# PRBonn/SHINE_mapping

Hardware: NVIDIA H100
Metric: sdf_train_points_per_sec_fwd_bwd (higher is better)
Workload: dtype f32

## Files before the change

### shine_mapping_b200/csrc/shine_b200.cu

```cuda

#include <cuda_runtime.h>
#include <math.h>
#include <stdint.h>

#include "shine_b200.h"

#ifndef SHINE_SECTOR_PROBE_TRAIN
#define SHINE_SECTOR_PROBE_TRAIN 0
#endif
#ifndef SHINE_SECTOR_PROBE_INFER
#define SHINE_SECTOR_PROBE_INFER 1
#endif
#ifndef SHINE_CPASYNC_PREFETCH
#define SHINE_CPASYNC_PREFETCH 0
#endif
#ifndef SHINE_GATHER_GROUP
#define SHINE_GATHER_GROUP 2
#endif
#ifndef SHINE_SLOT_PREFETCH
#define SHINE_SLOT_PREFETCH 0
#endif
#ifndef SHINE_ZERO_TILE_SKIP
#define SHINE_ZERO_TILE_SKIP 1
#endif
// ... 205 lines not shown
    }
    float g3[3] = {0.f, 0.f, 0.f};
    float4 acc = make_float4(0.f, 0.f, 0.f, 0.f);
    for (int i = 0; i < oct.num_levels; ++i) {
        const shine_level& lv = oct.lv[i];
        const HashSlot* slots = reinterpret_cast<const HashSlot*>(lv.hash_slots);
        const int s = valid ? probe_slot(slots, lv.hash_capacity - 1, morton_of(x, y, z, lv.level)) : -1;
        if (s < 0) continue;
        const int4 ia = ldg_i4(slots[s].ids0), ib = ldg_i4(slots[s].ids1);
        const int ids[8] = {ia.x, ib.x, ia.y, ib.y, ia.z, ib.z, ia.w, ib.w};
        BlendD b; b.init(x, y, z, lv.level, oct.poly_interp != 0);
#pragma unroll
        for (int c = 0; c < 8; ++c) {
            float g[3]; b.dw(c, g);
            if (MODE == 0) {
                const float4 v = ldg_f4(lv.features + (int64_t)ids[c] * F + 4 * part);
                const float q = v.x * d.x + v.y * d.y + v.z * d.z + v.w * d.w;
                g3[0] = fmaf(g[0], q, g3[0]); g3[1] = fmaf(g[1], q, g3[1]); g3[2] = fmaf(g[2], q, g3[2]);
            } else {
                const float w = tg[0] * g[0] + tg[1] * g[1] + tg[2] * g[2];
                if (MODE == 1) {
                    const float4 v = ldg_f4(lv.features + (int64_t)ids[c] * F + 4 * part);
                    acc.x = fmaf(w, v.x, acc.x); acc.y = fmaf(w, v.y, acc.y); acc.z = fmaf(w, v.z, acc.z); acc.w = fmaf(w, v.w, acc.w);
                } else {
                    red_add_f4(lv.feature_grads + (int64_t)ids[c] * F + 4 * part, w * d.x, w * d.y, w * d.z, w * d.w);
                }
            }
        }
    }
    if (MODE == 0) {
#pragma unroll
        for (int o = 1; o < LP; o <<= 1) {
            g3[0] += __shfl_xor_sync(kFull, g3[0], o); g3[1] += __shfl_xor_sync(kFull, g3[1], o); g3[2] += __shfl_xor_sync(kFull, g3[2], o);
        }
        if (valid && part == 0) { out[3 * p] = g3[0]; out[3 * p + 1] = g3[1]; out[3 * p + 2] = g3[2]; }
    } else if (MODE == 1) {
        if (valid) *reinterpret_cast<float4*>(out + p * F + 4 * part) = acc;
    }
}

__device__ __forceinline__ void to_afrag(const float (&v)[4], int odd, float (&a)[4]) {
    const float s0 = odd ? v[0] : v[2], s1 = odd ? v[1] : v[3];
    const float r0 = __shfl_xor_sync(kFull, s0, 1), r1 = __shfl_xor_sync(kFull, s1, 1);
    if (!odd) { a[0] = v[0]; a[2] = v[1]; a[1] = r0; a[3] = r1; }
    else      { a[0] = r0;   a[2] = r1;   a[1] = v[2]; a[3] = v[3]; }
}
__device__ __forceinline__ void from_cfrag(const float (&c)[4], int odd, float (&v)[4]) {
    const float s0 = odd ? c[0] : c[2], s1 = odd ? c[1] : c[3];
    const float r0 = __shfl_xor_sync(kFull, s0, 1), r1 = __shfl_xor_sync(kFull, s1, 1);
    if (!odd) { v[0] = c[0]; v[1] = c[1]; v[2] = r0; v[3] = r1; }
    else      { v[0] = r0;   v[1] = r1;   v[2] = c[2]; v[3] = c[3]; }
}

__device__ __forceinline__ void reduce_scatter_g(const float (&v)[24], float (&out)[3], int lane) {
    float a[12], b[6];
    const bool b4 = (lane & 16) != 0, b3 = (lane & 8) != 0, b2 = (lane & 4) != 0;
#pragma unroll
    for (int i = 0; i < 12; ++i) a[i] = (b4 ? v[12 + i] : v[i]) + __shfl_xor_sync(kFull, b4 ? v[i] : v[12 + i], 16);
#pragma unroll
    for (int i = 0; i < 6; ++i) b[i] = (b3 ? a[6 + i] : a[i]) + __shfl_xor_sync(kFull, b3 ? a[i] : a[6 + i], 8);
#pragma unroll
    for (int i = 0; i < 3; ++i) out[i] = (b2 ? b[3 + i] : b[i]) + __shfl_xor_sync(kFull, b2 ? b[i] : b[3 + i], 4);
}

#define SHINE_ACC_DECL float dW2[2][4][4], dW1[2][4], db2p[4][2], db1p[4][2], dw3p[4][2]

__device__ __forceinline__ void round_bar(int id) { asm volatile("bar.sync %0, 256;" ::"r"(id) : "memory"); }


constexpr int kGatherGroup = SHINE_GATHER_GROUP;

using shine_internal::StepParams;

struct SmemPlan {
    static constexpr int W1 = 0;
    static constexpr int W1T = W1 + 2 * kH * kF;
    static constexpr int W2 = W1T + 2 * kF * kWS;
    static constexpr int W2T = W2 + 2 * kH * kWS;
    static constexpr int B1 = W2T + 2 * kH * kWS;
    static constexpr int B2 = B1 + kH;
    static constexpr int W3 = B2 + kH;
    static constexpr int B3 = W3 + kH;
    static constexpr int kDecGradFloats = kH * kF + kH + kH * kH + kH + kH + 1;
    static constexpr int RND = B3 + 4;
    static constexpr int PRE = RND + 8;
    static constexpr int kPrePerWarp = 5 * kTile;
    static constexpr int STAGE = PRE + 8 * kPrePerWarp;
    static constexpr int kStagePerWarp = 3 * kTile * kWS + kTile * kF;
    static constexpr int kGroupPerLevel = 4 * kTile;
};

constexpr int kMaxGroupedRuns = 6;

__device__ __forceinline__ void red_add_f2(float* p, float a, float b) {
    asm volatile("red.global.add.v2.f32 [%0], {%1,%2};" ::"l"(p), "f"(a), "f"(b) : "memory");
}
__device__ __forceinline__ int group_slot(int p) { return 4 * (p & 3) + (p >> 2); }

template <int LMAX>
__device__ __forceinline__ void grouped_scatter(const StepParams& P, int L, int tile, const float* __restrict__ pt,
                                                float* __restrict__ dtile, const float (&dxc)[4], int lane) {
    const int g = lane >> 2, t = lane & 3;
    *reinterpret_cast<float2*>(dtile + g * kF + 2 * t) = make_float2(dxc[0], dxc[1]);
    *reinterpret_cast<float2*>(dtile + (g + 8) * kF + 2 * t) = make_float2(dxc[2], dxc[3]);
    __syncwarp();
    uint2 bh[2], bl[2];
#pragma unroll
    for (int c = 0; c < 2; ++c)
        split_fast2(dtile[(8 * c + t) * kF + g], dtile[(8 * c + t + 4) * kF + g], bh[c].x, bh[c].y, bl[c].x, bl[c].y);
    const float sx = (g & 4) ? 1.f : -1.f, ox = (g & 4) ? 0.f : 1.f;
    const float sy = (g & 2) ? 1.f : -1.f, oy = (g & 2) ? 0.f : 1.f;
    const float sz = (g & 1) ? 1.f : -1.f, oz = (g & 1) ? 0.f : 1.f;
    const int id_off = 8 * (g & 1) + 4 + (g >> 1);
    const int own = group_slot(lane & 15);
#pragma unroll
    for (int i = 0; i < LMAX; ++i) {
        if (i >= L) break;
        const float* lt = pt + i * SmemPlan::kGroupPerLevel;
        const int v_own = __float_as_int(lt[48 + own]);
        const uint32_t same = __match_any_sync(kFull, v_own);
        const int lead = __ffs(same) - 1;
        const uint32_t bmask = __ballot_sync(kFull, v_own >= 0 && lead == lane);
        if (bmask == 0) continue;
        const int rid_own = v_own >= 0 ? __popc(bmask & ((1u << lead) - 1u)) : 255;
        const shine_level& lv = P.oct.lv[i];
        const int32_t* slot_words = reinterpret_cast<const int32_t*>(lv.hash_slots);
        float* gb = grad_base(lv, (uint32_t)tile, kF);
        const int nruns = __popc(bmask);
        if (nruns > kMaxGroupedRuns) {
            const int odd = t & 1, half = t >> 1, mp = group_slot(g + 8 * odd);
            const int v = __float_as_int(lt[48 + mp]);
            if (v >= 0) {
                const float tx = lt[mp], ty = lt[16 + mp], tz = lt[32 + mp];
                const float ux = __fsub_rn(1.0f, tx), uy = __fsub_rn(1.0f, ty), uz = __fsub_rn(1.0f, tz);
                const int4 e = ldg_i4(slot_words + 16 * (int64_t)v + 4), o = ldg_i4(slot_words + 16 * (int64_t)v + 12);
                const int ids[8] = {e.x, o.x, e.y, o.y, e.z, o.z, e.w, o.w};
                const float4 d = *reinterpret_cast<const float4*>(dtile + (g + 8 * odd) * kF + 4 * half);
                const float xy[4] = {__fmul_rn(ux, uy), __fmul_rn(ux, ty), __fmul_rn(tx, uy), __fmul_rn(tx, ty)};
                const f2_t zz = f2_pack(uz, tz), d01 = f2_pack(d.x, d.y), d23 = f2_pack(d.z, d.w);
#pragma unroll
                for (int c = 0; c < 8; c += 2) {
// ... 29 lines not shown
        uint32_t rem = bmask;
        for (int r = 0; r < nruns; r += 2) {
            const int p1 = __ffs(rem) - 1; rem &= rem - 1;
            const int p2 = rem ? __ffs(rem) - 1 : p1; rem &= rem - 1;
            const int v1 = __shfl_sync(kFull, v_own, p1);
            const int v2 = (r + 1 < nruns) ? __shfl_sync(kFull, v_own, p2) : -1;
            AFrag<3> a0, a1;
            a0.set(rid[0] == r ? w[0] : 0.f, rid[0] == r + 1 ? w[0] : 0.f, rid[1] == r ? w[1] : 0.f, rid[1] == r + 1 ? w[1] : 0.f);
            a1.set(rid[2] == r ? w[2] : 0.f, rid[2] == r + 1 ? w[2] : 0.f, rid[3] == r ? w[3] : 0.f, rid[3] == r + 1 ? w[3] : 0.f);
            float c0[4] = {0.f, 0.f, 0.f, 0.f}, c1[4] = {0.f, 0.f, 0.f, 0.f};
            mma3x2<3>(c0, c1, a0, a1, bh[0], bl[0], bh[1], bl[1]);
            if (v1 >= 0) {
                const int row = __ldg(slot_words + 16 * (int64_t)v1 + id_off);
                red_add_f2(gb + (int64_t)row * kF + 2 * t, c0[0] + c1[0], c0[1] + c1[1]);
            }
            if (v2 >= 0) {
                const int row = __ldg(slot_words + 16 * (int64_t)v2 + id_off);
                red_add_f2(gb + (int64_t)row * kF + 2 * t, c0[2] + c1[2], c0[3] + c1[3]);
            }
        }
    }
    __syncwarp();
}

template <int NTF, bool TRAIN, bool DEC_GRAD, int LMAX, bool GROUPED = false>
__global__ void __launch_bounds__(256, !TRAIN ? SHINE_INFER_MINB : (DEC_GRAD && !GROUPED) ? SHINE_TRAIN_DECGRAD_MINB : SHINE_TRAIN_MINB)
sdf_fused_kernel(const __grid_constant__ StepParams P) {
    static_assert(!GROUPED || TRAIN, "the grouped scatter belongs to the training kernels");
    static_assert(!DEC_GRAD || TRAIN, "decoder gradients belong to the training kernels");
    static_assert(SmemPlan::kStagePerWarp >= SmemPlan::kDecGradFloats, "a warp's staging area holds its partial decoder gradient");
    extern __shared__ __align__(16) float smem[];
    uint32_t* smu = reinterpret_cast<uint32_t*>(smem);
    const int tid = threadIdx.x, lane = tid & 31, warp = tid >> 5;
    const int g = lane >> 2, t = lane & 3, odd = t & 1, half = t >> 1;
    constexpr int kWarps = 8;

    for (int i = tid; i < kH * kF; i += blockDim.x) {
        const int nrow = i / kF, k = i % kF;
        uint32_t hi, lo; split_tf32(P.dec.w1[i], hi, lo);
        smu[SmemPlan::W1 + i] = hi; smu[SmemPlan::W1 + kH * kF + i] = lo;
        smu[SmemPlan::W1T + k * kWS + nrow] = hi; smu[SmemPlan::W1T + kF * kWS + k * kWS + nrow] = lo;
    }
    for (int i = tid; i < kH * kH; i += blockDim.x) {
        const int nrow = i / kH, k = i % kH;
        uint32_t hi, lo; split_tf32(P.dec.w2[i], hi, lo);
        smu[SmemPlan::W2 + nrow * kWS + k] = hi; smu[SmemPlan::W2 + kH * kWS + nrow * kWS + k] = lo;
        smu[SmemPlan::W2T + k * kWS + nrow] = hi; smu[SmemPlan::W2T + kH * kWS + k * kWS + nrow] = lo;
    }
    if (tid < kH) {
        smem[SmemPlan::B1 + tid] = P.dec.b1 ? P.dec.b1[tid] : 0.f;
        smem[SmemPlan::B2 + tid] = P.dec.b2 ? P.dec.b2[tid] : 0.f;
        smem[SmemPlan::W3 + tid] = P.dec.w3[tid];
    }
    if (tid == 0) smem[SmemPlan::B3] = P.dec.b3 ? P.dec.b3[0] : 0.f;
    constexpr int kPark = LMAX <= 4 ? 16 : 32;
    constexpr int kIdPark = 4 * LMAX;
    __syncthreads();
    SHINE_ACC_DECL;
#pragma unroll
    for (int a = 0; a < 2; ++a) {
#pragma unroll
        for (int b = 0; b < 4; ++b) { dW2[a][b][0] = dW2[a][b][1] = dW2[a][b][2] = dW2[a][b][3] = 0.f; }
        dW1[a][0] = dW1[a][1] = dW1[a][2] = dW1[a][3] = 0.f;
    }
#pragma unroll
    for (int j = 0; j < 4; ++j) { db2p[j][0] = db2p[j][1] = db1p[j][0] = db1p[j][1] = dw3p[j][0] = dw3p[j][1] = 0.f; }
    float dW2acc[4] = {0.f, 0.f, 0.f, 0.f}, dW1acc[4] = {0.f, 0.f, 0.f, 0.f};
    float vecacc[3] = {0.f, 0.f, 0.f};
    constexpr bool kRounds = DEC_GRAD && GROUPED;

    constexpr bool kSectorProbe = TRAIN ? (SHINE_SECTOR_PROBE_TRAIN != 0) : (SHINE_SECTOR_PROBE_INFER != 0);
    constexpr bool kSlotPrefetch = TRAIN && !kSectorProbe && (SHINE_SLOT_PREFETCH != 0) && (SHINE_CPASYNC_PREFETCH == 0);
    constexpr bool kZeroSkip = (SHINE_ZERO_TILE_SKIP != 0) && (SHINE_CPASYNC_PREFETCH == 0);
    const bool poly = P.oct.poly_interp != 0;
    const int L = P.oct.num_levels;
    const float up = (TRAIN && P.d_loss) ? __ldg(P.d_loss) : 1.0f;
    const float gscale = P.loss_scale * up;

    float db3p = 0.f;
    float loss_acc = 0.f;

    float* stage = smem + SmemPlan::STAGE + warp * SmemPlan::kStagePerWarp;
    float* stA = stage;
    float* stB = stage + kTile * kWS;
    float* stC = stage + 2 * kTile * kWS;
    float* stX = stage + 3 * kTile * kWS;
    float* gpt = smem + SmemPlan::STAGE + (DEC_GRAD ? 8 * SmemPlan::kStagePerWarp : 0) +
                 warp * (LMAX * SmemPlan::kGroupPerLevel + (DEC_GRAD ? 0 : kTile * kF));
    float* gdx = DEC_GRAD ? stX : gpt + LMAX * SmemPlan::kGroupPerLevel;

    auto wgrad_round = [&](bool staged) {
        if (lane == 0) smu[SmemPlan::RND + warp] = staged ? 1u : 0u;
        round_bar(1);
        uint32_t present = 0;
#pragma unroll
        for (int v = 0; v < kWarps; ++v) present |= (smu[SmemPlan::RND + v] != 0u ? 1u : 0u) << v;
        const int mt = warp >> 2, nt = warp & 3;
#pragma unroll
        for (int v = 0; v < kWarps; ++v) {
            if (!((present >> v) & 1u)) continue;
            const float* sA = smem + SmemPlan::STAGE + v * SmemPlan::kStagePerWarp;
            const float* sB = sA + kTile * kWS;
#pragma unroll
            for (int ks = 0; ks < 2; ++ks) {
                uint2 bh, bl;
                split_fast2(sB[(8 * ks + t) * kWS + 8 * nt + g], sB[(8 * ks + t + 4) * kWS + 8 * nt + g], bh.x, bh.y, bl.x, bl.y);
                AFrag<NTF> a;
                a.set_packed(sA[(8 * ks + t) * kWS + 16 * mt + g], sA[(8 * ks + t) * kWS + 16 * mt + g + 8],
                             sA[(8 * ks + t + 4) * kWS + 16 * mt + g], sA[(8 * ks + t + 4) * kWS + 16 * mt + g + 8]);
                mma3<NTF>(dW2acc, a, bh, bl);
            }
        }
        const int m1 = warp & 1;
#pragma unroll
        for (int vv = 0; vv < 2; ++vv) {
            const int v = 2 * (warp >> 1) + vv;
            if (!((present >> v) & 1u)) continue;
            const float* sC = smem + SmemPlan::STAGE + v * SmemPlan::kStagePerWarp + 2 * kTile * kWS;
            const float* sX = sC + kTile * kWS;
#pragma unroll
            for (int ks = 0; ks < 2; ++ks) {
                uint2 bh, bl;
                split_fast2(sX[(8 * ks + t) * kF + g], sX[(8 * ks + t + 4) * kF + g], bh.x, bh.y, bl.x, bl.y);
                AFrag<NTF> a;
                a.set_packed(sC[(8 * ks + t) * kWS + 16 * m1 + g], sC[(8 * ks + t) * kWS + 16 * m1 + g + 8],
                             sC[(8 * ks + t + 4) * kWS + 16 * m1 + g], sC[(8 * ks + t + 4) * kWS + 16 * m1 + g + 8]);
                mma3<NTF>(dW1acc, a, bh, bl);
            }
        }
        round_bar(2);
    };

    const int warp_global = blockIdx.x * kWarps + warp;
    const int warp_stride = gridDim.x * kWarps;

    bool consecutive = true;
#pragma unroll
    for (int i = 1; i < LMAX; ++i)
        if (i < L && P.oct.lv[i].level != P.oct.lv[0].level - i) consecutive = false;

    unsigned long long skey0 = 0ull;
    int smine[LMAX / 2];
    uint4 skf[LMAX / 2];
#pragma unroll
    for (int j = 0; j < LMAX / 2; ++j) smine[j] = -1;
    auto stage_slots = [&](bool v, float sx, float sy, float sz) {
        skey0 = v ? morton_of(sx, sy, sz, P.oct.lv[0].level) : 0ull;
#pragma unroll
        for (int j = 0; j < LMAX / 2; ++j) {
            const int i = 2 * j + half;
            smine[j] = -1;
            if (i < L && v) {
                const shine_level& lv = P.oct.lv[i];
                const unsigned long long kq = consecutive ? (skey0 >> (3 * i)) : morton_of(sx, sy, sz, lv.level);
                smine[j] = (int)(hash_key(kq) & (lv.hash_capacity - 1));
                const HashSlot* sp = reinterpret_cast<const HashSlot*>(lv.hash_slots) + smine[j];
                if (SHINE_SLOT_PREFETCH == 2) {
                    skf[j] = __ldg(reinterpret_cast<const uint4*>(sp));
                } else {
                    asm volatile("prefetch.global.L1 [%0];" ::"l"(sp));
                    asm volatile("prefetch.global.L1 [%0];" ::"l"(reinterpret_cast<const char*>(sp) + 32));
                }
            }
        }
    };

    auto tile_of = [&](int seq) -> int {
        if constexpr (SHINE_PERMUTE_TILES != 0)
            return (P.tile_perm_mul > 1 && seq < P.num_tiles) ? (int)(((long long)seq * P.tile_perm_mul) % P.num_tiles) : seq;
        else
            return seq;
    };

#if SHINE_CPASYNC_PREFETCH
    float* pre = smem + SmemPlan::PRE + warp * SmemPlan::kPrePerWarp;
    const uint32_t pre_s = (uint32_t)__cvta_generic_to_shared(pre);
    auto prefetch_inputs = [&](int tl) {
        if (tl < P.num_tiles) {
            const int64_t base = (int64_t)tl * kTile;
            const int64_t left = P.n - base;
            const int npts = left < kTile ? (int)left : kTile;
#pragma unroll
            for (int r = 0; r < 3; ++r) {
// ... 1 lines not shown
                const float* src = nullptr;
                if (wd < 48) { if (wd < 3 * npts) src = P.coord + 3 * base + wd; }
                else if (wd < 64) { if (P.label && wd - 48 < npts) src = P.label + base + (wd - 48); }
                else if (wd < 80) { if (P.weighted && wd - 64 < npts) src = P.weight + base + (wd - 64); }
                if (src) asm volatile("cp.async.ca.shared.global [%0], [%1], 4;" ::"r"(pre_s + 4u * (uint32_t)wd), "l"(src) : "memory");
            }
        }
        asm volatile("cp.async.commit_group;" ::: "memory");
    };
    prefetch_inputs(warp_global);

    for (int tile = warp_global; tile - (kRounds ? warp : 0) < P.num_tiles; tile += warp_stride) {
        const int64_t base = (int64_t)tile * kTile;
        const int64_t myp = base + g + 8 * odd;
        asm volatile("cp.async.wait_group 0;" ::: "memory");
        __syncwarp();
        const bool valid = myp < P.n;
        float x = 0.f, y = 0.f, z = 0.f, lab = 0.f, wgt = 1.f;
        if (valid) {
            const int lp = g + 8 * odd;
            x = pre[3 * lp]; y = pre[3 * lp + 1]; z = pre[3 * lp + 2];
            if (P.label) lab = pre[48 + lp];
            if (P.weighted) wgt = fabsf(pre[64 + lp]);
        }
        __syncwarp();
        prefetch_inputs(tile + warp_stride);

#else
    float nx = 0.f, ny = 0.f, nz = 0.f, nlab = 0.f, nwgt = 1.f;
    bool nvalid = false;
    auto prefetch_inputs = [&](int tl) {
        const int64_t p = (int64_t)tile_of(tl) * kTile + g + 8 * odd;
        nvalid = tl < P.num_tiles && p < P.n;
        if (nvalid) {
            nx = __ldg(P.coord + 3 * p); ny = __ldg(P.coord + 3 * p + 1); nz = __ldg(P.coord + 3 * p + 2);
            if (P.label) nlab = __ldg(P.label + p);
            if (P.weighted) nwgt = fabsf(__ldg(P.weight + p));
        }
    };
    prefetch_inputs(warp_global);
    if (kSlotPrefetch) stage_slots(nvalid, nx, ny, nz);

    int phase = kZeroSkip ? 0 : 1;
    bool advance = false, last_pass = false;
    float pred0 = 0.f, zsum = 0.f;
    auto bce_point = [&](float pv, float lb, float wg, float& li, float& dp) {
        const float zt = __fdividef(1.0f, 1.0f + __expf(-__fdividef(lb, P.sigma)));
        const float e = __expf(-fabsf(pv));
        li = fmaxf(pv, 0.f) - pv * zt + __logf(1.0f + e);
        dp = 0.f;
        if (TRAIN) {
            const float rs = __fdividef(1.0f, 1.0f + e);
            const float sg = pv >= 0.f ? rs : e * rs;
            dp = (sg - zt) * wg * gscale;
        }
    };
    const bool dynamic = (SHINE_DYNAMIC_TILES != 0) && !kRounds && P.tile_counter != nullptr;
    int next_tile = 0, pending = 0;
    if (dynamic && lane == 0) pending = atomicAdd(P.tile_counter, 1);
    for (int seq = warp_global;; seq = !advance ? seq : (dynamic ? next_tile : seq + warp_stride)) {
        if (last_pass) break;
        const int tile = tile_of(seq);
        if (phase == 1 && seq - (kRounds ? warp : 0) >= P.num_tiles) {
            if constexpr (kZeroSkip && DEC_GRAD) {
#pragma unroll
                for (int o = 16; o > 0; o >>= 1) zsum += __shfl_xor_sync(kFull, zsum, o);
                if (lane == 0) smem[SmemPlan::PRE + warp] = zsum;
                __syncthreads();
                if (!kRounds && warp != 0) break;
                float tot = 0.f;
#pragma unroll
                for (int w = 0; w < kWarps; ++w) tot += smem[SmemPlan::PRE + w];
                if (tot == 0.f) break;
                zsum = tot;
                phase = 2;
            } else {
                break;
            }
        }
        const bool virt = phase != 1;
        last_pass = phase == 2;
        advance = !virt;
        if (kRounds && phase == 2 && warp != 0) { wgrad_round(false); continue; }
        const int64_t base = (int64_t)tile * kTile;
        const int64_t myp = base + g + 8 * odd;
        const bool valid = virt ? false : nvalid;
        const float x = nx, y = ny, z = nz, lab = nlab, wgt = nwgt;
        if (!virt) {
            if (dynamic) {
                next_tile = warp_stride + __shfl_sync(kFull, pending, 0);
                prefetch_inputs(next_tile);
                if (lane == 0) pending = atomicAdd(P.tile_counter, 1);
            } else {
                prefetch_inputs(seq + warp_stride);
            }
        }

#endif
        float feat[4];
        float pk[kPark];
        float idp[kIdPark];
        uint32_t hitmask = 0;
        if constexpr (kSectorProbe) {
        {
            float acc[8] = {0.f, 0.f, 0.f, 0.f, 0.f, 0.f, 0.f, 0.f};
#pragma unroll
            for (int i = 0; i < kPark; ++i) pk[i] = 0.f;
// ... 108 lines not shown
                    const int4 id4 = ldg_i4(slot_ids(slots, slot[i], half));
                    idp[4 * i] = __int_as_float(id4.x); idp[4 * i + 1] = __int_as_float(id4.y);
                    idp[4 * i + 2] = __int_as_float(id4.z); idp[4 * i + 3] = __int_as_float(id4.w);
                    float r0[8], r1[8], r2[8], r3[8];
                    ldg_row8(lv.features + (int64_t)id4.x * kF, r0);
                    ldg_row8(lv.features + (int64_t)id4.y * kF, r1);
                    ldg_row8(lv.features + (int64_t)id4.z * kF, r2);
                    ldg_row8(lv.features + (int64_t)id4.w * kF, r3);
                    Blend b; b.init(x, y, z, lv.level, poly);
                    pk[3 * i] = b.tx; pk[3 * i + 1] = b.ty; pk[3 * i + 2] = b.tz;
                    if (GROUPED) {
                        float* lt = gpt + i * SmemPlan::kGroupPerLevel + group_slot(g + 8 * odd);
                        if (half) lt[32] = b.tz; else { lt[0] = b.tx; lt[16] = b.ty; }
                    }
                    const float wz = half ? b.tz : b.uz;
                    const float w0 = __fmul_rn(__fmul_rn(b.ux, b.uy), wz), w1 = __fmul_rn(__fmul_rn(b.ux, b.ty), wz);
                    const float w2 = __fmul_rn(__fmul_rn(b.tx, b.uy), wz), w3 = __fmul_rn(__fmul_rn(b.tx, b.ty), wz);
                    blend4(acc, r0, r1, r2, r3, w0, w1, w2, w3);
                }
            }
#pragma unroll
            for (int q = 0; q < 4; ++q) {
                const float send = half ? acc[q] : acc[4 + q];
                const float recv = __shfl_xor_sync(kFull, send, 2);
                feat[q] = (half ? acc[4 + q] : acc[q]) + recv;
            }
        }
        }
#if !SHINE_CPASYNC_PREFETCH
        if (kZeroSkip && phase == 1 && __ballot_sync(kFull, hitmask != 0u) == 0u) {
            if (!TRAIN && P.mask && half == 0 && valid) P.mask[myp] = 0;
            if (P.pred && half == 0 && valid) P.pred[myp] = pred0;
            if (P.label != nullptr && valid) {
                float li, dpz;
                bce_point(pred0, lab, wgt, li, dpz);
                if (half == 0) { loss_acc += wgt * li; zsum += dpz; }
            }
            if (kRounds) wgrad_round(false);
            continue;
        }
#endif
        if (!TRAIN && P.mask) {
            bool present = false;
#pragma unroll
            for (int i = 0; i < LMAX; ++i) present = (i == P.mask_level) ? (((hitmask >> i) & 1u) != 0) : present;
            if (half == 0 && valid) P.mask[myp] = (uint8_t)present;
        }

        AFrag<NTF> ax;
        {
            float a[4]; to_afrag(feat, odd, a);
            ax.set(a[0], a[1], a[2], a[3]);
        }
        if (DEC_GRAD)
            *reinterpret_cast<float4*>(stX + (g + 8 * odd) * kF + 4 * half) = make_float4(feat[0], feat[1], feat[2], feat[3]);
        float h1[4][4];
        uint32_t m1 = 0;
        {
            uint2 bh[4], bl[4];
#pragma unroll
            for (int j = 0; j < 4; ++j) {
                const float bA = smem[SmemPlan::B1 + 8 * j + 2 * t], bB = smem[SmemPlan::B1 + 8 * j + 2 * t + 1];
                h1[j][0] = bA; h1[j][1] = bB; h1[j][2] = bA; h1[j][3] = bB;
                const int off = (8 * j + g) * kF + 2 * t;
                bh[j] = *reinterpret_cast<const uint2*>(smu + SmemPlan::W1 + off);
                bl[j] = *reinterpret_cast<const uint2*>(smu + SmemPlan::W1 + kH * kF + off);
            }
            mma3x4<NTF>(h1, ax, bh, bl);
#pragma unroll
            for (int j = 0; j < 4; ++j) {
#pragma unroll
                for (int r = 0; r < 4; ++r) {
                    if (TRAIN && h1[j][r] > 0.f) m1 |= 1u << (4 * j + r);
                    h1[j][r] = fmaxf(h1[j][r], 0.f);
                }
                if (DEC_GRAD) {
                    *reinterpret_cast<float2*>(stB + g * kWS + 8 * j + 2 * t) = make_float2(h1[j][0], h1[j][1]);
                    *reinterpret_cast<float2*>(stB + (g + 8) * kWS + 8 * j + 2 * t) = make_float2(h1[j][2], h1[j][3]);
                }
            }
        }
        float h2[4][4];
        {
#pragma unroll
            for (int j = 0; j < 4; ++j) {
                const float bA = smem[SmemPlan::B2 + 8 * j + 2 * t], bB = smem[SmemPlan::B2 + 8 * j + 2 * t + 1];
                h2[j][0] = bA; h2[j][1] = bB; h2[j][2] = bA; h2[j][3] = bB;
            }
#pragma unroll
            for (int kk = 0; kk < 4; ++kk) {
                AFrag<NTF> a; a.set(h1[kk][0], h1[kk][2], h1[kk][1], h1[kk][3]);
                uint2 bh[4], bl[4];
#pragma unroll
                for (int j = 0; j < 4; ++j) {
                    const int off = (8 * j + g) * kWS + 8 * kk + 2 * t;
                    bh[j] = *reinterpret_cast<const uint2*>(smu + SmemPlan::W2 + off);
                    bl[j] = *reinterpret_cast<const uint2*>(smu + SmemPlan::W2 + kH * kWS + off);
                }
                mma3x4<NTF>(h2, a, bh, bl);
            }
#pragma unroll
            for (int j = 0; j < 4; ++j) {
#pragma unroll
                for (int r = 0; r < 4; ++r) h2[j][r] = fmaxf(h2[j][r], 0.f);
            }
        }
        float w3a[4], w3b[4];
#pragma unroll
        for (int j = 0; j < 4; ++j) { w3a[j] = smem[SmemPlan::W3 + 8 * j + 2 * t]; w3b[j] = smem[SmemPlan::W3 + 8 * j + 2 * t + 1]; }
        float p0 = 0.f, p8 = 0.f;
#pragma unroll
        for (int j = 0; j < 4; ++j) {
            p0 = fmaf(h2[j][0], w3a[j], p0); p0 = fmaf(h2[j][1], w3b[j], p0);
            p8 = fmaf(h2[j][2], w3a[j], p8); p8 = fmaf(h2[j][3], w3b[j], p8);
        }
        p0 += __shfl_xor_sync(kFull, p0, 1); p0 += __shfl_xor_sync(kFull, p0, 2);
        p8 += __shfl_xor_sync(kFull, p8, 1); p8 += __shfl_xor_sync(kFull, p8, 2);
        const float b3 = smem[SmemPlan::B3];
        p0 += b3; p8 += b3;
        const float pown = odd ? p8 : p0;
#if !SHINE_CPASYNC_PREFETCH
        if (kZeroSkip && phase == 0) { pred0 = pown; phase = 1; continue; }
#endif
        if (P.pred && half == 0 && valid) P.pred[myp] = pown;

        if (P.label == nullptr) {
            if (kRounds) wgrad_round(false);
            continue;
        }

        float dpo = 0.f;
        if (valid) {
#if !SHINE_CPASYNC_PREFETCH
            float li;
            bce_point(pown, lab, wgt, li, dpo);
            if (half == 0) loss_acc += wgt * li;
#else
            const float zt = __fdividef(1.0f, 1.0f + __expf(-__fdividef(lab, P.sigma)));
            const float e = __expf(-fabsf(pown));
            const float li = fmaxf(pown, 0.f) - pown * zt + __logf(1.0f + e);
            if (half == 0) loss_acc += wgt * li;
            if (TRAIN) {
                const float rs = __fdividef(1.0f, 1.0f + e);
                const float sg = pown >= 0.f ? rs : e * rs;
                dpo = (sg - zt) * wgt * gscale;
            }
#endif
        }
        if (!TRAIN) continue;
#if !SHINE_CPASYNC_PREFETCH
        if (kZeroSkip && phase == 2) dpo = (g == 0 && odd == 0) ? zsum : 0.f;
#endif

        const float dpx = __shfl_xor_sync(kFull, dpo, 1);
        const float dp0 = odd ? dpx : dpo, dp8 = odd ? dpo : dpx;
        float dh2[4][4];
        float db2t[4][2], db1t[4][2], dw3t[4][2];
#pragma unroll
        for (int j = 0; j < 4; ++j) {
            dh2[j][0] = h2[j][0] > 0.f ? dp0 * w3a[j] : 0.f; dh2[j][1] = h2[j][1] > 0.f ? dp0 * w3b[j] : 0.f;
            dh2[j][2] = h2[j][2] > 0.f ? dp8 * w3a[j] : 0.f; dh2[j][3] = h2[j][3] > 0.f ? dp8 * w3b[j] : 0.f;
            if (DEC_GRAD) {
                dw3t[j][0] = dp0 * h2[j][0] + dp8 * h2[j][2];  dw3t[j][1] = dp0 * h2[j][1] + dp8 * h2[j][3];
                db2t[j][0] = dh2[j][0] + dh2[j][2];            db2t[j][1] = dh2[j][1] + dh2[j][3];
                *reinterpret_cast<float2*>(stA + g * kWS + 8 * j + 2 * t) = make_float2(dh2[j][0], dh2[j][1]);
                *reinterpret_cast<float2*>(stA + (g + 8) * kWS + 8 * j + 2 * t) = make_float2(dh2[j][2], dh2[j][3]);
            }
        }
        if (DEC_GRAD && t == 0) db3p += dp0 + dp8;

        float dh1[4][4];
        {
#pragma unroll
            for (int j = 0; j < 4; ++j) { dh1[j][0] = dh1[j][1] = dh1[j][2] = dh1[j][3] = 0.f; }
#pragma unroll
            for (int kk = 0; kk < 4; ++kk) {
                AFrag<NTF> a; a.set(dh2[kk][0], dh2[kk][2], dh2[kk][1], dh2[kk][3]);
                uint2 bh[4], bl[4];
#pragma unroll
                for (int j = 0; j < 4; ++j) {
                    const int off = (8 * j + g) * kWS + 8 * kk + 2 * t;
                    bh[j] = *reinterpret_cast<const uint2*>(smu + SmemPlan::W2T + off);
                    bl[j] = *reinterpret_cast<const uint2*>(smu + SmemPlan::W2T + kH * kWS + off);
                }
                mma3x4<NTF>(dh1, a, bh, bl);
            }
#pragma unroll
            for (int j = 0; j < 4; ++j) {
#pragma unroll
                for (int r = 0; r < 4; ++r) dh1[j][r] = ((m1 >> (4 * j + r)) & 1u) ? dh1[j][r] : 0.f;
                if (DEC_GRAD) {
                    db1t[j][0] = dh1[j][0] + dh1[j][2]; db1t[j][1] = dh1[j][1] + dh1[j][3];
                    *reinterpret_cast<float2*>(stC + g * kWS + 8 * j + 2 * t) = make_float2(dh1[j][0], dh1[j][1]);
                    *reinterpret_cast<float2*>(stC + (g + 8) * kWS + 8 * j + 2 * t) = make_float2(dh1[j][2], dh1[j][3]);
                }
            }
        }
        float dxc[4] = {0.f, 0.f, 0.f, 0.f};
        {
            float dxo[4] = {0.f, 0.f, 0.f, 0.f};
#pragma unroll
            for (int kk = 0; kk < 4; kk += 2) {
                AFrag<NTF> a0, a1;
                a0.set(dh1[kk][0], dh1[kk][2], dh1[kk][1], dh1[kk][3]);
                a1.set(dh1[kk + 1][0], dh1[kk + 1][2], dh1[kk + 1][1], dh1[kk + 1][3]);
                const int off = g * kWS + 8 * kk + 2 * t;
                const uint2 bh0 = *reinterpret_cast<const uint2*>(smu + SmemPlan::W1T + off);
                const uint2 bl0 = *reinterpret_cast<const uint2*>(smu + SmemPlan::W1T + kF * kWS + off);
                const uint2 bh1 = *reinterpret_cast<const uint2*>(smu + SmemPlan::W1T + off + 8);
                const uint2 bl1 = *reinterpret_cast<const uint2*>(smu + SmemPlan::W1T + kF * kWS + off + 8);
                mma3x2<NTF>(dxc, dxo, a0, a1, bh0, bl0, bh1, bl1);
            }
#pragma unroll
            for (int r = 0; r < 4; ++r) dxc[r] += dxo[r];
        }

        if (DEC_GRAD && !kRounds) {
#pragma unroll
            for (int j = 0; j < 4; ++j) {
                db2p[j][0] += db2t[j][0]; db2p[j][1] += db2t[j][1];
                db1p[j][0] += db1t[j][0]; db1p[j][1] += db1t[j][1];
                dw3p[j][0] += dw3t[j][0]; dw3p[j][1] += dw3t[j][1];
            }
            __syncwarp();
#pragma unroll
            for (int ks = 0; ks < 2; ++ks) {
                uint2 bh[4], bl[4];
#pragma unroll
                for (int nt = 0; nt < 4; ++nt) {
                    const float b0 = stB[(8 * ks + t) * kWS + 8 * nt + g], b1 = stB[(8 * ks + t + 4) * kWS + 8 * nt + g];
                    split_fast2(b0, b1, bh[nt].x, bh[nt].y, bl[nt].x, bl[nt].y);
                }
#pragma unroll
                for (int mt = 0; mt < 2; ++mt) {
                    AFrag<NTF> a;
                    a.set_packed(stA[(8 * ks + t) * kWS + 16 * mt + g], stA[(8 * ks + t) * kWS + 16 * mt + g + 8],
                          stA[(8 * ks + t + 4) * kWS + 16 * mt + g], stA[(8 * ks + t + 4) * kWS + 16 * mt + g + 8]);
                    mma3x4<NTF>(dW2[mt], a, bh, bl);
                }
            }
#pragma unroll
            for (int ks = 0; ks < 2; ++ks) {
                uint2 bh, bl;
                split_fast2(stX[(8 * ks + t) * kF + g], stX[(8 * ks + t + 4) * kF + g], bh.x, bh.y, bl.x, bl.y);
                AFrag<NTF> a0, a1;
                a0.set_packed(stC[(8 * ks + t) * kWS + g], stC[(8 * ks + t) * kWS + g + 8],
                              stC[(8 * ks + t + 4) * kWS + g], stC[(8 * ks + t + 4) * kWS + g + 8]);
                a1.set_packed(stC[(8 * ks + t) * kWS + 16 + g], stC[(8 * ks + t) * kWS + 16 + g + 8],
                              stC[(8 * ks + t + 4) * kWS + 16 + g], stC[(8 * ks + t + 4) * kWS + 16 + g + 8]);
                mma3x2<NTF>(dW1[0], dW1[1], a0, a1, bh, bl, bh, bl);
            }
            __syncwarp();
                }
        if (kRounds) {
            float cols[24];
#pragma unroll
            for (int j = 0; j < 4; ++j) {
#pragma unroll
                for (int q = 0; q < 2; ++q) { cols[2 * j + q] = db1t[j][q]; cols[8 + 2 * j + q] = db2t[j][q]; cols[16 + 2 * j + q] = dw3t[j][q]; }
            }
            float sums[3];
            reduce_scatter_g(cols, sums, lane);
#pragma unroll
            for (int i = 0; i < 3; ++i) vecacc[i] += sums[i];
            wgrad_round(true);
        }

#if !SHINE_CPASYNC_PREFETCH
        if (kSlotPrefetch) stage_slots(nvalid, nx, ny, nz);
#endif
        if constexpr (GROUPED) {
            static_assert(!GROUPED || !kSectorProbe, "the grouped scatter reads the node slots of the level-split walk");
            grouped_scatter<LMAX>(P, L, tile, gpt, gdx, dxc, lane);
            continue;
        }
        float dx[4];
        from_cfrag(dxc, odd, dx);
        const float (&qk)[kPark] = pk;
        const float (&qid)[kIdPark] = idp;
#pragma unroll
        for (int i = 0; i < LMAX; ++i) {
            int ids[8];
#pragma unroll
            for (int k = 0; k < 4; ++k) {
                const int mine = __float_as_int(qid[4 * i + k]);
                const int other = __shfl_xor_sync(kFull, mine, 2);
                ids[2 * k] = half ? other : mine;
                ids[2 * k + 1] = half ? mine : other;
            }
            if (i < L && ids[0] >= 0) {
                const shine_level& lv = P.oct.lv[i];
                Blend b;
                b.tx = qk[3 * i]; b.ty = qk[3 * i + 1]; b.tz = qk[3 * i + 2];
                b.ux = __fsub_rn(1.0f, b.tx); b.uy = __fsub_rn(1.0f, b.ty); b.uz = __fsub_rn(1.0f, b.tz);
                float* gb = grad_base(lv, (uint32_t)tile, kF) + 4 * half;
                const float xy[4] = {__fmul_rn(b.ux, b.uy), __fmul_rn(b.ux, b.ty), __fmul_rn(b.tx, b.uy), __fmul_rn(b.tx, b.ty)};
                const f2_t zz = f2_pack(b.uz, b.tz), dx01 = f2_pack(dx[0], dx[1]), dx23 = f2_pack(dx[2], dx[3]);
#pragma unroll
                for (int c = 0; c < 8; c += 2) {
                    float w[2];
                    f2_unpack(f2_mul(f2_pack(xy[c >> 1], xy[c >> 1]), zz), w[0], w[1]);
#pragma unroll
                    for (int k = 0; k < 2; ++k) {
                        const f2_t wk = f2_pack(w[k], w[k]);
                        float g0, g1, g2, g3;
                        f2_unpack(f2_mul(wk, dx01), g0, g1); f2_unpack(f2_mul(wk, dx23), g2, g3);
#if SHINE_EXPERIMENT_NO_RED
                        if (P.sigma == -12345.f)
#endif
                        red_add_f4(gb + (int64_t)ids[c + k] * kF, g0, g1, g2, g3);
                    }
                }
            }
        }
    }

    if (P.loss && P.label) {
#pragma unroll
        for (int o = 16; o > 0; o >>= 1) loss_acc += __shfl_xor_sync(kFull, loss_acc, o);
        if (lane == 0 && loss_acc != 0.f) atomicAdd(P.loss, loss_acc * P.loss_scale);
    }
    if (kRounds) {
        {
            const int mt = warp >> 2, nt = warp & 3;
#pragma unroll
            for (int r = 0; r < 4; ++r)
                if (dW2acc[r] != 0.f) atomicAdd(P.dec.gw2 + (16 * mt + g + 8 * (r >> 1)) * kH + 8 * nt + 2 * t + (r & 1), dW2acc[r]);
        }
        float* part = stage;
        constexpr int oB1 = 128, oB3 = 224, kParts = 225;
        *reinterpret_cast<float2*>(part + g * kF + 2 * t) = make_float2(dW1acc[0], dW1acc[1]);
        *reinterpret_cast<float2*>(part + (g + 8) * kF + 2 * t) = make_float2(dW1acc[2], dW1acc[3]);
#pragma unroll
        for (int i = 0; i < 3; ++i) {
            const int s = 3 * g + i, k = s >> 3, j = (s & 7) >> 1, q = s & 1;
            part[oB1 + 32 * k + 8 * j + 2 * t + q] = vecacc[i];
        }
#pragma unroll
        for (int o = 16; o > 0; o >>= 1) db3p += __shfl_xor_sync(kFull, db3p, o);
        if (lane == 0) part[oB3] = db3p;
        __syncthreads();
        for (int i = tid; i < 2 * oB1 + (kParts - oB1); i += blockDim.x) {
            float v = 0.f;
            float* dst;
            if (i < 2 * oB1) {
                const int m = i / oB1, e = i % oB1;
#pragma unroll
                for (int c = 0; c < kWarps / 2; ++c) v += smem[SmemPlan::STAGE + (2 * c + m) * SmemPlan::kStagePerWarp + e];
                dst = P.dec.gw1 + 16 * m * kF + e;
            } else {
                const int e = i - oB1;
#pragma unroll
                for (int w = 0; w < kWarps; ++w) v += smem[SmemPlan::STAGE + w * SmemPlan::kStagePerWarp + e];
                if (e < oB1 + kH) dst = P.dec.gb1 ? P.dec.gb1 + (e - oB1) : nullptr;
                else if (e < oB1 + 2 * kH) dst = P.dec.gb2 ? P.dec.gb2 + (e - oB1 - kH) : nullptr;
                else if (e < oB3) dst = P.dec.gw3 + (e - oB1 - 2 * kH);
                else dst = P.dec.gb3;
            }
            if (v != 0.f && dst) atomicAdd(dst, v);
        }
    }
    if (DEC_GRAD && !kRounds) {
        float* part = stage;
        constexpr int oW1 = 0, oB1 = 256, oW2 = 288, oB2 = 1312, oW3 = 1344, oB3 = 1376;
        __syncwarp();
#pragma unroll
        for (int mt = 0; mt < 2; ++mt) {
#pragma unroll
            for (int nt = 0; nt < 4; ++nt) {
                *reinterpret_cast<float2*>(part + oW2 + (16 * mt + g) * kH + 8 * nt + 2 * t) = make_float2(dW2[mt][nt][0], dW2[mt][nt][1]);
                *reinterpret_cast<float2*>(part + oW2 + (16 * mt + g + 8) * kH + 8 * nt + 2 * t) = make_float2(dW2[mt][nt][2], dW2[mt][nt][3]);
            }
            *reinterpret_cast<float2*>(part + oW1 + (16 * mt + g) * kF + 2 * t) = make_float2(dW1[mt][0], dW1[mt][1]);
            *reinterpret_cast<float2*>(part + oW1 + (16 * mt + g + 8) * kF + 2 * t) = make_float2(dW1[mt][2], dW1[mt][3]);
        }
#pragma unroll
        for (int j = 0; j < 4; ++j) {
#pragma unroll
            for (int q = 0; q < 2; ++q) {
                float a = db1p[j][q], b = db2p[j][q], c = dw3p[j][q];
#pragma unroll
                for (int o = 4; o < 32; o <<= 1) {
                    a += __shfl_xor_sync(kFull, a, o); b += __shfl_xor_sync(kFull, b, o); c += __shfl_xor_sync(kFull, c, o);
                }
                if (g == 0) {
                    part[oB1 + 8 * j + 2 * t + q] = a;
                    part[oB2 + 8 * j + 2 * t + q] = b;
                    part[oW3 + 8 * j + 2 * t + q] = c;
                }
            }
        }
#pragma unroll
        for (int o = 16; o > 0; o >>= 1) db3p += __shfl_xor_sync(kFull, db3p, o);
        if (lane == 0) part[oB3] = db3p;
        __syncthreads();
        for (int i = tid; i < SmemPlan::kDecGradFloats; i += blockDim.x) {
            float v = 0.f;
#pragma unroll
            for (int w = 0; w < kWarps; ++w) v += smem[SmemPlan::STAGE + w * SmemPlan::kStagePerWarp + i];
            if (v == 0.f) continue;
            float* dst;
            if (i < oB1) dst = P.dec.gw1 + i;
// ... 694 lines not shown
```

Baseline: 3.721 billion.

## Stage weight-grad operands in fragment-swizzled layout and split rounds into half-block barriers

Per-warp staging buffers for dh2, h1, dh1 and features are rewritten into a swizzled MMA-fragment layout, so operand loads become single float4/float2 reads instead of scattered scalar reads with padded strides. The cross-warp weight-gradient round now splits the K dimension across two 128-thread halves with separate named barriers, and each warp computes two N-tiles. The db1/db2 bias reductions are folded into the round from the staged A fragments instead of a 24-wide shuffle reduce-scatter. gscale moves to shared memory. This cuts shared-memory bank conflicts, shuffle count and barrier width, but adds a more complex final reduction of dW2 partials through shared memory and extra smem reads for gscale.

```diff
diff --git a/shine_mapping_b200/csrc/shine_b200.cu b/shine_mapping_b200/csrc/shine_b200.cu
--- a/shine_mapping_b200/csrc/shine_b200.cu
+++ b/shine_mapping_b200/csrc/shine_b200.cu
@@ -281,20 +281,41 @@
     else      { v[0] = r0;   v[1] = r1;   v[2] = c[2]; v[3] = c[3]; }
 }
 
-__device__ __forceinline__ void reduce_scatter_g(const float (&v)[24], float (&out)[3], int lane) {
-    float a[12], b[6];
+#define SHINE_ACC_DECL float dW2[2][4][4], dW1[2][4], db2p[4][2], db1p[4][2], dw3p[4][2]
+
+__device__ __forceinline__ float reduce_scatter_g8(const float (&v)[8], int lane) {
+    float a[4], b[2];
     const bool b4 = (lane & 16) != 0, b3 = (lane & 8) != 0, b2 = (lane & 4) != 0;
 #pragma unroll
-    for (int i = 0; i < 12; ++i) a[i] = (b4 ? v[12 + i] : v[i]) + __shfl_xor_sync(kFull, b4 ? v[i] : v[12 + i], 16);
-#pragma unroll
-    for (int i = 0; i < 6; ++i) b[i] = (b3 ? a[6 + i] : a[i]) + __shfl_xor_sync(kFull, b3 ? a[i] : a[6 + i], 8);
-#pragma unroll
-    for (int i = 0; i < 3; ++i) out[i] = (b2 ? b[3 + i] : b[i]) + __shfl_xor_sync(kFull, b2 ? b[i] : b[3 + i], 4);
-}
-
-#define SHINE_ACC_DECL float dW2[2][4][4], dW1[2][4], db2p[4][2], db1p[4][2], dw3p[4][2]
-
-__device__ __forceinline__ void round_bar(int id) { asm volatile("bar.sync %0, 256;" ::"r"(id) : "memory"); }
+    for (int i = 0; i < 4; ++i) a[i] = (b4 ? v[4 + i] : v[i]) + __shfl_xor_sync(kFull, b4 ? v[i] : v[4 + i], 16);
+#pragma unroll
+    for (int i = 0; i < 2; ++i) b[i] = (b3 ? a[2 + i] : a[i]) + __shfl_xor_sync(kFull, b3 ? a[i] : a[2 + i], 8);
+    return (b2 ? b[1] : b[0]) + __shfl_xor_sync(kFull, b2 ? b[0] : b[1], 4);
+}
+__device__ __forceinline__ void round_bar(int id) { asm volatile("bar.sync %0, 128;" ::"r"(id) : "memory"); }
+
+__device__ __forceinline__ int frag_chunk(int lane) { return lane ^ ((lane >> 2) & 6); }
+template <int NTF>
+__device__ __forceinline__ void load_afrag(const float* blk, int c, AFrag<NTF>& a) {
+    const float4 v = *reinterpret_cast<const float4*>(blk + 4 * c);
+    a.set_packed(v.x, v.y, v.z, v.w);
+}
+__device__ __forceinline__ void load_bfrag(const float* blk, int c, uint2& bh, uint2& bl) {
+    const float2 v = *reinterpret_cast<const float2*>(blk + 2 * c);
+    split_fast2(v.x, v.y, bh.x, bh.y, bl.x, bl.y);
+}
+__device__ __forceinline__ void stage_afrags(float* blk, const int (&sq)[2], const float (&c)[4][4]) {
+#pragma unroll
+    for (int mt = 0; mt < 2; ++mt)
+#pragma unroll
+        for (int q = 0; q < 2; ++q)
+            *reinterpret_cast<float4*>(blk + 128 * mt + 4 * sq[q]) = make_float4(c[2 * mt][q], c[2 * mt + 1][q], c[2 * mt][2 + q], c[2 * mt + 1][2 + q]);
+}
+__device__ __forceinline__ int xfrag_word(int ks, int c) { return 64 * ks + 2 * (c ^ (8 * ks)); }
+__device__ __forceinline__ void load_xfrag(const float* sx, int ks, int c, uint2& bh, uint2& bl) {
+    const float2 v = *reinterpret_cast<const float2*>(sx + xfrag_word(ks, c));
+    split_fast2(v.x, v.y, bh.x, bh.y, bl.x, bl.y);
+}
 
 
 constexpr int kGatherGroup = SHINE_GATHER_GROUP;
@@ -310,12 +331,17 @@
     static constexpr int B2 = B1 + kH;
     static constexpr int W3 = B2 + kH;
     static constexpr int B3 = W3 + kH;
+    static constexpr int GSCALE = B3 + 1;
     static constexpr int kDecGradFloats = kH * kF + kH + kH * kH + kH + kH + 1;
     static constexpr int RND = B3 + 4;
     static constexpr int PRE = RND + 8;
     static constexpr int kPrePerWarp = 5 * kTile;
     static constexpr int STAGE = PRE + 8 * kPrePerWarp;
-    static constexpr int kStagePerWarp = 3 * kTile * kWS + kTile * kF;
+    static constexpr int SA2 = 0;
+    static constexpr int SB2 = SA2 + kTile * kH;
+    static constexpr int SA1 = SB2 + kTile * kH;
+    static constexpr int SX = SA1 + kTile * kH;
+    static constexpr int kStagePerWarp = SX + kTile * kF;
     static constexpr int kGroupPerLevel = 4 * kTile;
 };
 
@@ -451,7 +477,10 @@
         smem[SmemPlan::B2 + tid] = P.dec.b2 ? P.dec.b2[tid] : 0.f;
         smem[SmemPlan::W3 + tid] = P.dec.w3[tid];
     }
-    if (tid == 0) smem[SmemPlan::B3] = P.dec.b3 ? P.dec.b3[0] : 0.f;
+    if (tid == 0) {
+        smem[SmemPlan::B3] = P.dec.b3 ? P.dec.b3[0] : 0.f;
+        smem[SmemPlan::GSCALE] = P.loss_scale * ((TRAIN && P.d_loss) ? __ldg(P.d_loss) : 1.0f);
+    }
     constexpr int kPark = LMAX <= 4 ? 16 : 32;
     constexpr int kIdPark = 4 * LMAX;
     __syncthreads();
@@ -464,8 +493,8 @@
     }
 #pragma unroll
     for (int j = 0; j < 4; ++j) { db2p[j][0] = db2p[j][1] = db1p[j][0] = db1p[j][1] = dw3p[j][0] = dw3p[j][1] = 0.f; }
-    float dW2acc[4] = {0.f, 0.f, 0.f, 0.f}, dW1acc[4] = {0.f, 0.f, 0.f, 0.f};
-    float vecacc[3] = {0.f, 0.f, 0.f};
+    float dW2acc[2][4] = {{0.f, 0.f, 0.f, 0.f}, {0.f, 0.f, 0.f, 0.f}}, dW1acc[4] = {0.f, 0.f, 0.f, 0.f};
+    float dw3acc = 0.f, db2acc[2] = {0.f, 0.f}, db1acc[2] = {0.f, 0.f};
     constexpr bool kRounds = DEC_GRAD && GROUPED;
 
     constexpr bool kSectorProbe = TRAIN ? (SHINE_SECTOR_PROBE_TRAIN != 0) : (SHINE_SECTOR_PROBE_INFER != 0);
@@ -473,61 +502,59 @@
     constexpr bool kZeroSkip = (SHINE_ZERO_TILE_SKIP != 0) && (SHINE_CPASYNC_PREFETCH == 0);
     const bool poly = P.oct.poly_interp != 0;
     const int L = P.oct.num_levels;
-    const float up = (TRAIN && P.d_loss) ? __ldg(P.d_loss) : 1.0f;
-    const float gscale = P.loss_scale * up;
 
     float db3p = 0.f;
     float loss_acc = 0.f;
 
     float* stage = smem + SmemPlan::STAGE + warp * SmemPlan::kStagePerWarp;
-    float* stA = stage;
-    float* stB = stage + kTile * kWS;
-    float* stC = stage + 2 * kTile * kWS;
-    float* stX = stage + 3 * kTile * kWS;
+    float* stX = stage + SmemPlan::SX;
+    const int kp = g >> 2, fc = frag_chunk(lane);
+    const int sq[2] = {frag_chunk(8 * t + (g & 3)), frag_chunk(8 * t + 4 + (g & 3))};
     float* gpt = smem + SmemPlan::STAGE + (DEC_GRAD ? 8 * SmemPlan::kStagePerWarp : 0) +
                  warp * (LMAX * SmemPlan::kGroupPerLevel + (DEC_GRAD ? 0 : kTile * kF));
     float* gdx = DEC_GRAD ? stX : gpt + LMAX * SmemPlan::kGroupPerLevel;
 
     auto wgrad_round = [&](bool staged) {
         if (lane == 0) smu[SmemPlan::RND + warp] = staged ? 1u : 0u;
-        round_bar(1);
+        round_bar(1 + 2 * (threadIdx.x >> 7));
         uint32_t present = 0;
 #pragma unroll
         for (int v = 0; v < kWarps; ++v) present |= (smu[SmemPlan::RND + v] != 0u ? 1u : 0u) << v;
-        const int mt = warp >> 2, nt = warp & 3;
-#pragma unroll
-        for (int v = 0; v < kWarps; ++v) {
+        const int mt = warp & 1, np = (warp >> 1) & 1, kh = warp >> 2;
+#pragma unroll
+        for (int i = 0; i < kWarps / 2; ++i) {
+            const int v = 4 * kh + i;
             if (!((present >> v) & 1u)) continue;
-            const float* sA = smem + SmemPlan::STAGE + v * SmemPlan::kStagePerWarp;
-            const float* sB = sA + kTile * kWS;
+            const float* s = smem + SmemPlan::STAGE + v * SmemPlan::kStagePerWarp;
 #pragma unroll
             for (int ks = 0; ks < 2; ++ks) {
-                uint2 bh, bl;
-                split_fast2(sB[(8 * ks + t) * kWS + 8 * nt + g], sB[(8 * ks + t + 4) * kWS + 8 * nt + g], bh.x, bh.y, bl.x, bl.y);
+                uint2 bh[2], bl[2];
+#pragma unroll
+                for (int n = 0; n < 2; ++n) load_bfrag(s + SmemPlan::SB2 + (4 * ks + 2 * np + n) * 64, fc, bh[n], bl[n]);
                 AFrag<NTF> a;
-                a.set_packed(sA[(8 * ks + t) * kWS + 16 * mt + g], sA[(8 * ks + t) * kWS + 16 * mt + g + 8],
-                             sA[(8 * ks + t + 4) * kWS + 16 * mt + g], sA[(8 * ks + t + 4) * kWS + 16 * mt + g + 8]);
-                mma3<NTF>(dW2acc, a, bh, bl);
-            }
-        }
-        const int m1 = warp & 1;
+                const float4 av = *reinterpret_cast<const float4*>(s + SmemPlan::SA2 + (2 * ks + mt) * 128 + 4 * fc);
+                a.set_packed(av.x, av.y, av.z, av.w);
+                if (np == 0) { db2acc[0] += av.x + av.z; db2acc[1] += av.y + av.w; }
+                mma3x2<NTF>(dW2acc[0], dW2acc[1], a, a, bh[0], bl[0], bh[1], bl[1]);
+            }
+        }
 #pragma unroll
         for (int vv = 0; vv < 2; ++vv) {
             const int v = 2 * (warp >> 1) + vv;
             if (!((present >> v) & 1u)) continue;
-            const float* sC = smem + SmemPlan::STAGE + v * SmemPlan::kStagePerWarp + 2 * kTile * kWS;
-            const float* sX = sC + kTile * kWS;
+            const float* s = smem + SmemPlan::STAGE + v * SmemPlan::kStagePerWarp;
 #pragma unroll
             for (int ks = 0; ks < 2; ++ks) {
                 uint2 bh, bl;
-                split_fast2(sX[(8 * ks + t) * kF + g], sX[(8 * ks + t + 4) * kF + g], bh.x, bh.y, bl.x, bl.y);
+                load_xfrag(s + SmemPlan::SX, ks, fc, bh, bl);
                 AFrag<NTF> a;
-                a.set_packed(sC[(8 * ks + t) * kWS + 16 * m1 + g], sC[(8 * ks + t) * kWS + 16 * m1 + g + 8],
-                             sC[(8 * ks + t + 4) * kWS + 16 * m1 + g], sC[(8 * ks + t + 4) * kWS + 16 * m1 + g + 8]);
+                const float4 av = *reinterpret_cast<const float4*>(s + SmemPlan::SA1 + (2 * ks + mt) * 128 + 4 * fc);
+                a.set_packed(av.x, av.y, av.z, av.w);
+                db1acc[0] += av.x + av.z; db1acc[1] += av.y + av.w;
                 mma3<NTF>(dW1acc, a, bh, bl);
             }
         }
-        round_bar(2);
+        round_bar(2 + 2 * (threadIdx.x >> 7));
     };
 
     const int warp_global = blockIdx.x * kWarps + warp;
@@ -635,7 +662,7 @@
         if (TRAIN) {
             const float rs = __fdividef(1.0f, 1.0f + e);
             const float sg = pv >= 0.f ? rs : e * rs;
-            dp = (sg - zt) * wg * gscale;
+            dp = (sg - zt) * wg * smem[SmemPlan::GSCALE];
         }
     };
     const bool dynamic = (SHINE_DYNAMIC_TILES != 0) && !kRounds && P.tile_counter != nullptr;
@@ -850,8 +877,10 @@
             float a[4]; to_afrag(feat, odd, a);
             ax.set(a[0], a[1], a[2], a[3]);
         }
-        if (DEC_GRAD)
-            *reinterpret_cast<float4*>(stX + (g + 8 * odd) * kF + 4 * half) = make_float4(feat[0], feat[1], feat[2], feat[3]);
+        if (DEC_GRAD) {
+#pragma unroll
+            for (int q = 0; q < 4; ++q) stX[xfrag_word(kp, frag_chunk(16 * half + 4 * q + (g & 3))) + odd] = feat[q];
+        }
         float h1[4][4];
         uint32_t m1 = 0;
         {
@@ -873,8 +902,9 @@
                     h1[j][r] = fmaxf(h1[j][r], 0.f);
                 }
                 if (DEC_GRAD) {
-                    *reinterpret_cast<float2*>(stB + g * kWS + 8 * j + 2 * t) = make_float2(h1[j][0], h1[j][1]);
-                    *reinterpret_cast<float2*>(stB + (g + 8) * kWS + 8 * j + 2 * t) = make_float2(h1[j][2], h1[j][3]);
+#pragma unroll
+                    for (int q = 0; q < 2; ++q)
+                        *reinterpret_cast<float2*>(stage + SmemPlan::SB2 + (4 * kp + j) * 64 + 2 * sq[q]) = make_float2(h1[j][q], h1[j][2 + q]);
                 }
             }
         }
@@ -941,7 +971,7 @@
             if (TRAIN) {
                 const float rs = __fdividef(1.0f, 1.0f + e);
                 const float sg = pown >= 0.f ? rs : e * rs;
-                dpo = (sg - zt) * wgt * gscale;
+                dpo = (sg - zt) * wgt * smem[SmemPlan::GSCALE];
             }
 #endif
         }
@@ -961,10 +991,9 @@
             if (DEC_GRAD) {
                 dw3t[j][0] = dp0 * h2[j][0] + dp8 * h2[j][2];  dw3t[j][1] = dp0 * h2[j][1] + dp8 * h2[j][3];
                 db2t[j][0] = dh2[j][0] + dh2[j][2];            db2t[j][1] = dh2[j][1] + dh2[j][3];
-                *reinterpret_cast<float2*>(stA + g * kWS + 8 * j + 2 * t) = make_float2(dh2[j][0], dh2[j][1]);
-                *reinterpret_cast<float2*>(stA + (g + 8) * kWS + 8 * j + 2 * t) = make_float2(dh2[j][2], dh2[j][3]);
-            }
-        }
+            }
+        }
+        if (DEC_GRAD) stage_afrags(stage + SmemPlan::SA2 + 256 * kp, sq, dh2);
         if (DEC_GRAD && t == 0) db3p += dp0 + dp8;
 
         float dh1[4][4];
@@ -987,12 +1016,9 @@
             for (int j = 0; j < 4; ++j) {
 #pragma unroll
                 for (int r = 0; r < 4; ++r) dh1[j][r] = ((m1 >> (4 * j + r)) & 1u) ? dh1[j][r] : 0.f;
-                if (DEC_GRAD) {
-                    db1t[j][0] = dh1[j][0] + dh1[j][2]; db1t[j][1] = dh1[j][1] + dh1[j][3];
-                    *reinterpret_cast<float2*>(stC + g * kWS + 8 * j + 2 * t) = make_float2(dh1[j][0], dh1[j][1]);
-                    *reinterpret_cast<float2*>(stC + (g + 8) * kWS + 8 * j + 2 * t) = make_float2(dh1[j][2], dh1[j][3]);
-                }
-            }
+                if (DEC_GRAD) { db1t[j][0] = dh1[j][0] + dh1[j][2]; db1t[j][1] = dh1[j][1] + dh1[j][3]; }
+            }
+            if (DEC_GRAD) stage_afrags(stage + SmemPlan::SA1 + 256 * kp, sq, dh1);
         }
         float dxc[4] = {0.f, 0.f, 0.f, 0.f};
         {
@@ -1025,42 +1051,30 @@
             for (int ks = 0; ks < 2; ++ks) {
                 uint2 bh[4], bl[4];
 #pragma unroll
-                for (int nt = 0; nt < 4; ++nt) {
-                    const float b0 = stB[(8 * ks + t) * kWS + 8 * nt + g], b1 = stB[(8 * ks + t + 4) * kWS + 8 * nt + g];
-                    split_fast2(b0, b1, bh[nt].x, bh[nt].y, bl[nt].x, bl[nt].y);
-                }
+                for (int nt = 0; nt < 4; ++nt) load_bfrag(stage + SmemPlan::SB2 + (4 * ks + nt) * 64, fc, bh[nt], bl[nt]);
 #pragma unroll
                 for (int mt = 0; mt < 2; ++mt) {
                     AFrag<NTF> a;
-                    a.set_packed(stA[(8 * ks + t) * kWS + 16 * mt + g], stA[(8 * ks + t) * kWS + 16 * mt + g + 8],
-                          stA[(8 * ks + t + 4) * kWS + 16 * mt + g], stA[(8 * ks + t + 4) * kWS + 16 * mt + g + 8]);
+                    load_afrag(stage + SmemPlan::SA2 + (2 * ks + mt) * 128, fc, a);
                     mma3x4<NTF>(dW2[mt], a, bh, bl);
                 }
             }
 #pragma unroll
             for (int ks = 0; ks < 2; ++ks) {
                 uint2 bh, bl;
-                split_fast2(stX[(8 * ks + t) * kF + g], stX[(8 * ks + t + 4) * kF + g], bh.x, bh.y, bl.x, bl.y);
+                load_xfrag(stX, ks, fc, bh, bl);
                 AFrag<NTF> a0, a1;
-                a0.set_packed(stC[(8 * ks + t) * kWS + g], stC[(8 * ks + t) * kWS + g + 8],
-                              stC[(8 * ks + t + 4) * kWS + g], stC[(8 * ks + t + 4) * kWS + g + 8]);
-                a1.set_packed(stC[(8 * ks + t) * kWS + 16 + g], stC[(8 * ks + t) * kWS + 16 + g + 8],
-                              stC[(8 * ks + t + 4) * kWS + 16 + g], stC[(8 * ks + t + 4) * kWS + 16 + g + 8]);
+                load_afrag(stage + SmemPlan::SA1 + (2 * ks) * 128, fc, a0);
+                load_afrag(stage + SmemPlan::SA1 + (2 * ks + 1) * 128, fc, a1);
                 mma3x2<NTF>(dW1[0], dW1[1], a0, a1, bh, bl, bh, bl);
             }
             __syncwarp();
-                }
+        }
         if (kRounds) {
-            float cols[24];
-#pragma unroll
-            for (int j = 0; j < 4; ++j) {
-#pragma unroll
-                for (int q = 0; q < 2; ++q) { cols[2 * j + q] = db1t[j][q]; cols[8 + 2 * j + q] = db2t[j][q]; cols[16 + 2 * j + q] = dw3t[j][q]; }
-            }
-            float sums[3];
-            reduce_scatter_g(cols, sums, lane);
-#pragma unroll
-            for (int i = 0; i < 3; ++i) vecacc[i] += sums[i];
+            float cols[8];
+#pragma unroll
+            for (int j = 0; j < 4; ++j) { cols[2 * j] = dw3t[j][0]; cols[2 * j + 1] = dw3t[j][1]; }
+            dw3acc += reduce_scatter_g8(cols, lane);
             wgrad_round(true);
         }
 
@@ -1119,26 +1133,35 @@
         if (lane == 0 && loss_acc != 0.f) atomicAdd(P.loss, loss_acc * P.loss_scale);
     }
     if (kRounds) {
-        {
-            const int mt = warp >> 2, nt = warp & 3;
-#pragma unroll
-            for (int r = 0; r < 4; ++r)
-                if (dW2acc[r] != 0.f) atomicAdd(P.dec.gw2 + (16 * mt + g + 8 * (r >> 1)) * kH + 8 * nt + 2 * t + (r & 1), dW2acc[r]);
-        }
         float* part = stage;
-        constexpr int oB1 = 128, oB3 = 224, kParts = 225;
+        constexpr int oB1 = 128, oB3 = 224, kParts = 225, oW2 = 256, kW2Block = 16 * 16;
+#pragma unroll
+        for (int n = 0; n < 2; ++n) {
+            *reinterpret_cast<float2*>(part + oW2 + g * 16 + 8 * n + 2 * t) = make_float2(dW2acc[n][0], dW2acc[n][1]);
+            *reinterpret_cast<float2*>(part + oW2 + (g + 8) * 16 + 8 * n + 2 * t) = make_float2(dW2acc[n][2], dW2acc[n][3]);
+        }
         *reinterpret_cast<float2*>(part + g * kF + 2 * t) = make_float2(dW1acc[0], dW1acc[1]);
         *reinterpret_cast<float2*>(part + (g + 8) * kF + 2 * t) = make_float2(dW1acc[2], dW1acc[3]);
-#pragma unroll
-        for (int i = 0; i < 3; ++i) {
-            const int s = 3 * g + i, k = s >> 3, j = (s & 7) >> 1, q = s & 1;
-            part[oB1 + 32 * k + 8 * j + 2 * t + q] = vecacc[i];
+        part[oB1 + 2 * kH + 8 * (g >> 1) + 2 * t + (g & 1)] = dw3acc;
+        {
+            const int mt = warp & 1, np = (warp >> 1) & 1;
+#pragma unroll
+            for (int r = 0; r < 2; ++r) {
+                float d1 = db1acc[r], d2 = db2acc[r];
+#pragma unroll
+                for (int o = 1; o < 4; o <<= 1) { d1 += __shfl_xor_sync(kFull, d1, o); d2 += __shfl_xor_sync(kFull, d2, o); }
+                if (t == 0) {
+                    part[oB1 + 16 * mt + g + 8 * r] = d1;           part[oB1 + 16 * (1 - mt) + g + 8 * r] = 0.f;
+                    part[oB1 + kH + 16 * mt + g + 8 * r] = np == 0 ? d2 : 0.f;   part[oB1 + kH + 16 * (1 - mt) + g + 8 * r] = 0.f;
+                }
+            }
         }
 #pragma unroll
         for (int o = 16; o > 0; o >>= 1) db3p += __shfl_xor_sync(kFull, db3p, o);
         if (lane == 0) part[oB3] = db3p;
         __syncthreads();
-        for (int i = tid; i < 2 * oB1 + (kParts - oB1); i += blockDim.x) {
+        constexpr int kVecEnd = 2 * oB1 + (kParts - oB1);
+        for (int i = tid; i < kVecEnd + 4 * kW2Block; i += blockDim.x) {
             float v = 0.f;
             float* dst;
             if (i < 2 * oB1) {
@@ -1146,6 +1169,11 @@
 #pragma unroll
                 for (int c = 0; c < kWarps / 2; ++c) v += smem[SmemPlan::STAGE + (2 * c + m) * SmemPlan::kStagePerWarp + e];
                 dst = P.dec.gw1 + 16 * m * kF + e;
+            } else if (i >= kVecEnd) {
+                const int b = (i - kVecEnd) / kW2Block, e = (i - kVecEnd) % kW2Block;
+                const float* p0 = smem + SmemPlan::STAGE + b * SmemPlan::kStagePerWarp + oW2 + e;
+                v = p0[0] + p0[4 * SmemPlan::kStagePerWarp];
+                dst = P.dec.gw2 + (16 * (b & 1) + e / 16) * kH + 16 * (b >> 1) + e % 16;
             } else {
                 const int e = i - oB1;
 #pragma unroll
```

Result: faster. 3.858 billion, median of 6 (+3.7%).
